# OATML-Markslab/ProteinGym

Measured on AMD Instinct MI355X. Metric: mutants scored/sec (ESM-1v 650M masked-marginal), higher is better.
Workload: dtype f16x3 (fp32 operands split into 2 fp16 planes, 3 fp16 MFMAs per product, fp32 accumulate)

## Files before the change

### proteingym_amd/csrc/api_ops.hip

```cpp
#include "model.h"

static inline float rebuild_split(unsigned short h, unsigned short l) {
    _Float16 a, b;
    memcpy(&a, &h, 2); memcpy(&b, &l, 2);
    return (float)a + (float)b * (1.0f / kLoScale);
}

extern "C" {

int pgmi_op_layernorm(int device, const float* x, const float* w, const float* b, int rows, int D, float eps, float* y) {
    if (!x || !w || !b || !y || rows <= 0 || D <= 0 || D % 4) { set_error("bad argument"); return PGMI_EINVAL; }
    if (pgmi_device_count() <= 0) { set_error("no HIP device visible"); return PGMI_ENODEV; }
    PGMI_HIP(hipSetDevice(device));
    std::vector<void*> pool;
    float *dx, *dw, *db, *dy;
    int rc = 0;
    if ((rc = dev_upload(pool, &dx, x, (size_t)rows * D)) || (rc = dev_upload(pool, &dw, w, (size_t)D)) ||
        (rc = dev_upload(pool, &db, b, (size_t)D)) || (rc = dev_alloc(pool, &dy, (size_t)rows * D))) {
        for (void* p : pool) hipFree(p);
        return rc;
    }
    launch_layernorm(dx, dw, db, rows, D, eps, dy, nullptr);
    hipError_t e = hipMemcpy(y, dy, (size_t)rows * D * 4, hipMemcpyDeviceToHost);
    for (void* p : pool) hipFree(p);
// ... 84 lines not shown
    if (er != hipSuccess) { set_error("moe op failed: %s", hipGetErrorString(er)); return PGMI_EHIP; }
    return PGMI_OK;
}

static GemmLaunch op_gemm(const unsigned short* a16, const W16& w16, const float* bias, int M, int N, int K, int variant) {
    GemmLaunch g;
    g.A = a16; g.W = w16.p; g.out_scale = w16.out_scale;
    g.bias = bias;
    g.M = M; g.N = N; g.K = K;
    g.variant = variant;
    return g;
}

int pgmi_op_gemm(int device, int precision, const float* A, const float* W, const float* bias, const float* residual,
                 int M, int N, int K, int epilogue, float* C) {
    if (!A || !W || !C || M <= 0 || N <= 0 || K <= 0) { set_error("bad argument"); return PGMI_EINVAL; }
    if (precision != PGMI_PREC_FP32 && precision != PGMI_PREC_F16X3 && precision != PGMI_PREC_BF16) { set_error("unknown precision %d", precision); return PGMI_EINVAL; }
    if (pgmi_device_count() <= 0) { set_error("no HIP device visible"); return PGMI_ENODEV; }
    PGMI_HIP(hipSetDevice(device));
    gemm_options_from_env();
    std::vector<void*> pool;
    float *dA, *dW = nullptr, *dB = nullptr, *dR = nullptr, *dC;
    int rc = 0;
    if ((rc = dev_upload(pool, &dA, A, (size_t)M * K)) ||
        (precision == PGMI_PREC_FP32 && (rc = dev_upload(pool, &dW, W, (size_t)N * K))) ||
        (bias && (rc = dev_upload(pool, &dB, bias, (size_t)N))) ||
        (residual && (rc = dev_upload(pool, &dR, residual, (size_t)M * N))) ||
        (rc = dev_alloc(pool, &dC, (size_t)M * N))) {
        for (void* p : pool) hipFree(p);
        return rc;
    }
    const int epi = epilogue & 255;
    const bool split_planes = (epilogue & 256) != 0;
    if (epi == EPI_SWIGLU && (!split_planes || precision != PGMI_PREC_F16X3 || (N % 64))) {
        for (void* p : pool) hipFree(p);
        set_error("SwiGLU GEMM op: precision f16x3 with the split-plane output (epilogue 4 + 256), N %% 64 == 0");
        return PGMI_EINVAL;
    }
    if (epi == EPI_RELU && precision != PGMI_PREC_F16X3) {
        for (void* p : pool) hipFree(p);
        set_error("ReLU GEMM op: precision f16x3 only");
        return PGMI_EINVAL;
    }
    if (split_planes && (precision == PGMI_PREC_FP32 || residual || (N % (precision == PGMI_PREC_F16X3 ? 32 : 4)))) {
        for (void* p : pool) hipFree(p);
        set_error("16-bit-plane GEMM op: f16x3 (N %% 32 == 0) or bf16 (N %% 4 == 0), no residual");
        return PGMI_EINVAL;
    }
    if (precision == PGMI_PREC_FP32) {
        rc = launch_gemm_f32(dA, dW, dB, dR, dC, M, N, K, epi, nullptr);
    } else {
        const bool bf = precision == PGMI_PREC_BF16;
        const int planes = bf ? 1 : 2;
        W16 w16;
        unsigned short* a16 = nullptr;
        rc = make_w16(pool, W, (size_t)N * K, (size_t)K, precision, nullptr, &w16);
        if (!rc) rc = dev_alloc(pool, &a16, (size_t)M * K * planes);
        if (!rc) {
            launch_split16(dA, (int64_t)M * K, 1.0f, bf ? 1 : 2, K, a16, nullptr);
            GemmLaunch g = op_gemm(a16, w16, dB, M, N, K, env_int("PGMI_GEMM_VARIANT", 0));
            g.epilogue = epi; g.bf = bf;
            if (split_planes) {
                unsigned short* c16 = nullptr;
                const int No = epi == EPI_SWIGLU ? N / 2 : N;
                rc = dev_alloc(pool, &c16, (size_t)M * N * 2);
                g.out16 = c16;
                if (!rc) rc = launch_gemm16(g);
                if (!rc) {
                    std::vector<unsigned short> h((size_t)M * N * 2);
                    hipError_t e2 = hipMemcpy(h.data(), c16, h.size() * 2, hipMemcpyDeviceToHost);
                    if (e2 != hipSuccess) { set_error("gemm op failed: %s", hipGetErrorString(e2)); rc = PGMI_EHIP; }
                    for (size_t m = 0; m < (size_t)M && !rc && bf; ++m)
                        for (int n = 0; n < N; ++n) {
                            const unsigned int u = (unsigned int)h[m * N + n] << 16;
                            memcpy(&C[m * N + n], &u, 4);
                        }
                    for (size_t m = 0; m < (size_t)M && !rc && !bf; ++m)
                        for (int n = 0; n < No; ++n) {
                            const size_t o = ki_off(m, n, No);
                            C[m * No + n] = rebuild_split(h[o], h[o + 32]);
                        }
                }
                for (void* p : pool) hipFree(p);
                return rc;
            }
            g.residual = dR; g.out32 = dC;
            rc = launch_gemm16(g);
        }
    }
    hipError_t e = hipMemcpy(C, dC, (size_t)M * N * 4, hipMemcpyDeviceToHost);
    for (void* p : pool) hipFree(p);
    if (rc) return rc;
    if (e != hipSuccess) { set_error("gemm op failed: %s", hipGetErrorString(e)); return PGMI_EHIP; }
    return PGMI_OK;
}

int pgmi_bench_gemm_ab(int device, int precision, int M, int N, int K, int epilogue, int split_out, const int* variants,
                       int n_variants, int rounds, int iters, double* ms_out) {
    if (M <= 0 || N <= 0 || K <= 0 || iters <= 0 || rounds <= 0 || n_variants <= 0 || !variants || !ms_out) { set_error("bad argument"); return PGMI_EINVAL; }
    if (pgmi_device_count() <= 0) { set_error("no HIP device visible"); return PGMI_ENODEV; }
    PGMI_HIP(hipSetDevice(device));
    gemm_options_from_env();
    std::vector<void*> pool;
    auto cleanup = [&]() { for (void* p : pool) hipFree(p); };
    std::vector<float> hA((size_t)M * K), hW((size_t)N * K), hb(N);
    unsigned int st = 12345u;
    auto rnd = [&]() { st = st * 1664525u + 1013904223u; return ((st >> 8) * (1.0f / 8388608.0f)) - 1.0f; };
    for (auto& v : hA) v = rnd();
    for (auto& v : hW) v = rnd() * 0.03f;
    for (auto& v : hb) v = rnd();
    float *dA, *dW = nullptr, *dB, *dC = nullptr;
    unsigned short *a16 = nullptr, *c16 = nullptr;
    int rc = 0;
    if ((rc = dev_upload(pool, &dA, hA.data(), hA.size())) || (rc = dev_upload(pool, &dB, hb.data(), hb.size()))) { cleanup(); return rc; }
    hipEvent_t e0, e1;
    PGMI_HIP(hipEventCreate(&e0));
// ... 674 lines not shown
```

### proteingym_amd/csrc/gemm16x_kernel.h

```cpp
#pragma once
#include <type_traits>

#include "common.h"

namespace pgmi {

typedef _Float16 h8 __attribute__((ext_vector_type(8)));
typedef _Float16 h4 __attribute__((ext_vector_type(4)));
typedef __bf16 b8 __attribute__((ext_vector_type(8)));
typedef unsigned int u32x4 __attribute__((ext_vector_type(4)));
typedef unsigned int u32x2 __attribute__((ext_vector_type(2)));

__device__ __forceinline__ f32x4 gelu_erf16(f32x4 x) {
    auto all = [](float v) { return f32x4{v, v, v, v}; };
    const f32x4 b = __builtin_elementwise_max(-__builtin_elementwise_abs(x), all(-6.0f));
    f32x4 q = __builtin_elementwise_fma(x, all(0.0f), all(3.309269596e-05f));
    q = __builtin_elementwise_fma(q, b, all(7.692188374e-04f));
    q = __builtin_elementwise_fma(q, b, all(8.080714382e-03f));
    q = __builtin_elementwise_fma(q, b, all(5.341210216e-02f));
    q = __builtin_elementwise_fma(q, b, all(-4.587709904e-01f));
    q = __builtin_elementwise_fma(q, b, all(1.151201725e+00f));
    q = __builtin_elementwise_fma(q, b, all(-9.999930859e-01f));
    const f32x4 e = {__builtin_amdgcn_exp2f(q[0]), __builtin_amdgcn_exp2f(q[1]), __builtin_amdgcn_exp2f(q[2]), __builtin_amdgcn_exp2f(q[3])};
    return __builtin_elementwise_fma(b, e, __builtin_elementwise_max(x, all(0.0f)));
// ... 128 lines not shown
            const int nwg = all_half ? n_items : tp.n_main, xcd = item & 7, q = nwg >> 3, r8 = nwg & 7;
            wgid = (xcd < r8 ? xcd * (q + 1) : r8 * (q + 1) + (xcd - r8) * q) + (item >> 3);
        } else {
            wgid = tp.n_main + ((item - tp.n_main) >> 1);
        }
        batch = 0;
        if (xm.tiles_per_batch) {
            batch = wgid / xm.tiles_per_batch;
            wgid -= batch * xm.tiles_per_batch;
            const int bi = batch % xm.batch_inner, bo = batch / xm.batch_inner;
            a_base = __builtin_amdgcn_readfirstlane((unsigned int)bi * xm.a_b0 + (unsigned int)bo * xm.a_b1);
            w_base = __builtin_amdgcn_readfirstlane((unsigned int)bi * xm.w_b0 + (unsigned int)bo * xm.w_b1);
            batch = __builtin_amdgcn_readfirstlane(batch);
        }
        int tm, tn;
        x_tile_coords(wgid, tp.tiles_m, tp.tiles_n, tm, tn, tp.group_m);
        half_item = all_half || (tp.half && item >= tp.n_main);
        a_ld = half_item ? LD / 2 : LD;
        m0 = __builtin_amdgcn_readfirstlane(all_half ? tm * (XBM / 2) : tm * XBM + (half_item ? ((item - tp.n_main) & 1) * (XBM / 2) : 0));
        n0 = __builtin_amdgcn_readfirstlane(tn * XBN);
#pragma unroll
        for (int i = 0; i < LD; ++i) {
            a_off[i] = (unsigned int)min(m0 + row_lo + 64 * i, M - 1) * a_row_bytes + (unsigned int)csrc * 16u;
            w_off[i] = (unsigned int)min(n0 + row_lo + 64 * i, N - 1) * w_row_bytes + (unsigned int)csrc * 16u;
        }
    };
    auto issue_tile = [&](int kt, int buf) {
        u32x4* base = lds + buf * X_STAGE + wave * 64;
        const int run = kt >> xm.k_run_log2, in_run = kt - (run << xm.k_run_log2);
        const int ka = (int)(a_base + (xm.a_run_bytes ? (unsigned int)run * xm.a_run_bytes + (unsigned int)in_run * 128u : (unsigned int)kt * 128u));
        const int kw = (int)(w_base + (xm.w_run_bytes ? (unsigned int)run * xm.w_run_bytes + (unsigned int)in_run * 128u : (unsigned int)kt * 128u));
#pragma unroll
        for (int i = 0; i < LD; ++i)
            if (i < a_ld)
                __builtin_amdgcn_raw_ptr_buffer_load_lds(rsA, (__attribute__((address_space(3))) void*)(base + XNT * i), 16, (int)a_off[i], ka, 0, 0);
#pragma unroll
        for (int i = 0; i < LD; ++i)
            __builtin_amdgcn_raw_ptr_buffer_load_lds(rsW, (__attribute__((address_space(3))) void*)(base + X_OP_CH + XNT * i), 16, (int)w_off[i], kw, 0, 0);
    };
    auto phase = [&]() {
        __builtin_amdgcn_sched_barrier(0);
        __builtin_amdgcn_s_waitcnt(0xC07F);
        __builtin_amdgcn_s_barrier();
        __builtin_amdgcn_sched_barrier(0);
    };
    auto phase_vm = [&]() {
        __builtin_amdgcn_sched_barrier(0);
        __builtin_amdgcn_s_waitcnt(0x0070);
        __builtin_amdgcn_s_barrier();
        __builtin_amdgcn_sched_barrier(0);
    };

    f32x4 acc[TN][TMX];
    u32x4 af[2][TMX / 2], wf[2][TN], whs[TN];
    const int fsw = (r >> 1) & 7;
    auto read_frags = [&](auto tmc, auto hc, const u32x4* Ab, const u32x4* Wb) {
        constexpr int TM = decltype(tmc)::value, TH = TM / 2, H = decltype(hc)::value;
// ... 38 lines not shown
#pragma unroll
        for (int j = 0; j < TN; ++j)
#pragma unroll
            for (int i = 0; i < TH; ++i) acc[j][H * TH + i] = mfma16x16<false>(whs[j], af[1][i], acc[j][H * TH + i]);
#pragma unroll
        for (int j = 0; j < TN; ++j)
#pragma unroll
            for (int i = 0; i < TH; ++i) acc[j][H * TH + i] = mfma16x16<false>(wf[0][j], af[0][i], acc[j][H * TH + i]);
        if constexpr (H == 0) {
#pragma unroll
            for (int k = 0; k < 4 * TN; ++k) {
                __builtin_amdgcn_sched_group_barrier(0x008, 1, 0);
                __builtin_amdgcn_sched_group_barrier(0x002, 1, 0);
            }
            __builtin_amdgcn_sched_group_barrier(0x008, 3 * TN * TH - 4 * TN, 0);
        }
    };
    using H0 = std::integral_constant<int, 0>;
    using H1 = std::integral_constant<int, 1>;

    int item = blockIdx.x;
    if (item >= n_items) return;
    decode(item);
    issue_tile(0, 0);
    auto run_item = [&](auto tmc) -> bool {
        constexpr int TM = decltype(tmc)::value;
        phase_vm();
#pragma unroll
        for (int j = 0; j < TN; ++j)
#pragma unroll
            for (int i = 0; i < TM; ++i)
#pragma unroll
                for (int v = 0; v < 4; ++v) acc[j][i][v] = 0.0f;
        int cur = 0;
        if (late) phase();
        for (int kt = 0; kt < nk; ++kt) {
            const u32x4* Ab = lds + cur * X_STAGE;
            const u32x4* Wb = Ab + X_OP_CH;
            __builtin_amdgcn_s_setprio(0);
            if (kt + 1 < nk) issue_tile(kt + 1, cur ^ 1);
            read_frags(tmc, H0{}, Ab, Wb);
            phase();
            __builtin_amdgcn_s_setprio(1);
            mfmas(tmc, H0{});
            phase();
            __builtin_amdgcn_s_setprio(0);
            read_frags(tmc, H1{}, Ab, Wb);
            if (late) phase_vm(); else phase();
            __builtin_amdgcn_s_setprio(1);
            mfmas(tmc, H1{});
            if (!late) phase_vm(); else phase();
            cur ^= 1;
        }
        __builtin_amdgcn_s_setprio(0);
        if (!late) phase();

        const int em0 = m0, en0 = n0, eb = batch;
        item += gridDim.x;
        const bool more = item < n_items;
        if (more) {
            decode(item);
            issue_tile(0, 0);
        }

        if constexpr (OUT == 2) {
            const int Dm = N / 3;
            const int nb = en0 + wn * 64;
            if (nb < N) {
            const int which = nb / Dm, hcol = nb - which * Dm, hh = hcol >> 6;
            constexpr int SPQ = 144;
            unsigned char* patch_q = patches + wave * (2 * 32 * SPQ);
            const bool staged_q = which < 2;
            f32x4 bq0[2], bq1[2];
#pragma unroll
            for (int g = 0; g < 2; ++g) {
                bq0[g] = *reinterpret_cast<const f32x4*>(bias + nb + 16 * g + 4 * kq);
                bq1[g] = *reinterpret_cast<const f32x4*>(bias + nb + 32 + 16 * g + 4 * kq);
            }
#pragma unroll
            for (int g = 0; g < 2; ++g) asm volatile("" :: "v"(bq0[g]), "v"(bq1[g]));
#pragma unroll
            for (int ib = 0; ib < TM / 2; ++ib) {
#pragma unroll
            for (int s = 0; s < 2; ++s) {
                const int i = 2 * ib + s, prow = 16 * s + r;
                const int m = em0 + (wm * TM + i) * 16 + r;
                const bool row_ok = m < M;
                if (!row_ok) continue;
                const int bb = m / qo.T, t = m - bb * qo.T;
                f32x4 rc[2], rs[2];
                if (which < 2 && qo.rotary) {
                    const int tr = (min(t, qo.T - 1) * qo.rot_halves + (hh % qo.rot_halves)) * 64;
#pragma unroll
                    for (int g = 0; g < 2; ++g) {
                        rc[g] = *reinterpret_cast<const f32x4*>(qo.cos_t + tr + 16 * g + 4 * kq);
                        rs[g] = *reinterpret_cast<const f32x4*>(qo.sin_t + tr + 16 * g + 4 * kq);
                    }
                }
#pragma unroll
                for (int g = 0; g < 2; ++g) {
                    const int d0 = 16 * g + 4 * kq;
// ... 47 lines not shown
                            c1p[0] = __builtin_bit_cast(unsigned short, a1);
                            c1p[qo.vt_plane] = __builtin_bit_cast(unsigned short, l1);
                        }
                    }
                }
            }
                if (staged_q) {
                    __builtin_amdgcn_wave_barrier();
                    const int m_base = em0 + (wm * TM + 2 * ib) * 16;
#pragma unroll
                    for (int k = 0; k < 4; ++k) {
                        const int q = lane + 64 * k, row = q >> 3, cc = q & 7;
                        const u32x4 vh = *reinterpret_cast<const u32x4*>(patch_q + row * SPQ + cc * 16);
                        const u32x4 vl = *reinterpret_cast<const u32x4*>(patch_q + (32 + row) * SPQ + cc * 16);
                        if (m_base + row < M) {
                            unsigned short* dst = Ch + (size_t)(m_base + row) * (2 * Dm) + (size_t)which * Dm + hcol + cc * 8;
                            *reinterpret_cast<u32x4*>(dst) = vh;
                            *reinterpret_cast<u32x4*>(dst + c_plane) = vl;
                        }
                    }
                    __builtin_amdgcn_wave_barrier();
                }
            }
            }
        } else if constexpr (OUT == 0) {
            unsigned char* patch = patches + wave * (32 * 128);
            const int cc = lane & 7, rq = lane >> 3;
            const unsigned int kOob = 0x80000000u;
            const unsigned int ldc = xm.ldc ? (unsigned int)xm.ldc : (unsigned int)N;
            const long long cb = xm.tiles_per_batch ? (long long)(eb % xm.batch_inner) * xm.c_b0 + (long long)(eb / xm.batch_inner) * xm.c_b1 : 0;
            const __amdgpu_buffer_rsrc_t rsC = __builtin_amdgcn_make_buffer_rsrc(Cf + cb, 0, (int)((unsigned int)M * ldc * 4u), 0x00020000);
            const __amdgpu_buffer_rsrc_t rsR = __builtin_amdgcn_make_buffer_rsrc(const_cast<float*>(residual ? residual : Cf) + cb, 0, (int)((unsigned int)M * ldc * 4u), 0x00020000);
            constexpr int NB = TN / 2;
            unsigned int coff[NB];
            f32x4 bv[NB];
#pragma unroll
            for (int j = 0; j < NB; ++j) {
                const int n = en0 + wn * 64 + j * 32 + cc * 4;
                coff[j] = n < N ? (unsigned int)n * 4u : kOob;
                bv[j] = (bias && n < N) ? *reinterpret_cast<const f32x4*>(bias + n) : f32x4{0.f, 0.f, 0.f, 0.f};
            }
#pragma unroll
            for (int j = 0; j < NB; ++j) asm volatile("" :: "v"(bv[j]));
            auto c_off = [&](int m, int j) -> int {
                return (int)((m < M && coff[j] != kOob) ? (unsigned int)m * ldc * 4u + coff[j] : kOob);
            };
            u32x4 rv[2][NB][4];
            auto load_residual = [&](int i, u32x4 (&dst)[NB][4]) {
                const int m_base = em0 + (wm * TM + 2 * i) * 16;
#pragma unroll
                for (int j = 0; j < NB; ++j)
#pragma unroll
                    for (int k = 0; k < 4; ++k)
                        dst[j][k] = __builtin_bit_cast(u32x4, __builtin_amdgcn_raw_buffer_load_b128(rsR, c_off(m_base + rq + 8 * k, j), 0, 0));
            };
            if (residual) load_residual(0, rv[0]);
#pragma unroll
            for (int i = 0; i < TM / 2; ++i) {
                const int m_base = em0 + (wm * TM + 2 * i) * 16;
                if (residual && i + 1 < TM / 2) load_residual(i + 1, rv[(i + 1) & 1]);
#pragma unroll
                for (int j = 0; j < NB; ++j) {
#pragma unroll
                    for (int s = 0; s < 2; ++s)
#pragma unroll
                        for (int u = 0; u < 2; ++u) {
                            const int prow = 16 * s + r;
                            *reinterpret_cast<f32x4*>(patch + prow * 128 + (((4 * u + kq) ^ (prow & 7)) << 4)) = acc[2 * j + u][2 * i + s];
                        }
                    __builtin_amdgcn_wave_barrier();
#pragma unroll
                    for (int k = 0; k < 4; ++k) {
                        const int row = rq + 8 * k;
                        const f32x4 a = *reinterpret_cast<const f32x4*>(patch + row * 128 + ((cc ^ (row & 7)) << 4));
                        f32x4 val;
#pragma unroll
                        for (int e = 0; e < 4; ++e) val[e] = fmaf(a[e], out_scale, bv[j][e]);
                        if (EPI == EPI_GELU) val = gelu_erf16(val);
                        if (EPI == EPI_GELU_TANH) val = gelu_tanh16(val);
                        if (EPI == EPI_SQRELU)
#pragma unroll
                        for (int e = 0; e < 4; ++e) { const float t = fmaxf(val[e], 0.0f); val[e] = t * t; }
                        if (EPI == EPI_RELU)
#pragma unroll
                        for (int e = 0; e < 4; ++e) val[e] = fmaxf(val[e], 0.0f);
                        if (residual) {
                            const f32x4 rr = __builtin_bit_cast(f32x4, rv[i & 1][j][k]);
#pragma unroll
                            for (int e = 0; e < 4; ++e) val[e] = rr[e] + val[e];
                        }
                        __builtin_amdgcn_raw_buffer_store_b128(__builtin_bit_cast(u32x4, val), rsC, c_off(m_base + row, j), 0, 0);
                    }
                    __builtin_amdgcn_wave_barrier();
                }
            }
        } else {
            if constexpr (BF) {
                constexpr int SPB = 144;
                const bool staged = (N % 8 == 0) && (en0 + (wn + 1) * 64 <= N);
                unsigned char* patch = patches + wave * (32 * SPB);
                f32x4 bvs[TN];
#pragma unroll
                for (int j = 0; j < TN; ++j) {
                    const int n = en0 + wn * 64 + 16 * j + 4 * kq;
                    bvs[j] = (bias && n < N) ? *reinterpret_cast<const f32x4*>(bias + n) : f32x4{0.f, 0.f, 0.f, 0.f};
                }
#pragma unroll
                for (int j = 0; j < TN; ++j) asm volatile("" :: "v"(bvs[j]));
#pragma unroll
                for (int ib = 0; ib < TM / 2; ++ib) {
#pragma unroll
                    for (int s = 0; s < 2; ++s) {
                    const int i = 2 * ib + s, prow = 16 * s + r;
                    const int m = em0 + (wm * TM + i) * 16 + r;
                    if (m >= M) continue;
#pragma unroll
                    for (int j = 0; j < TN; ++j) {
                            const int n = en0 + wn * 64 + 16 * j + 4 * kq;
                            if (n >= N) continue;
                            const f32x4 bv = bvs[j];
                            f32x4 val;
#pragma unroll
                            for (int e = 0; e < 4; ++e) val[e] = fmaf(acc[j][i][e], out_scale, bv[e]);
                            if (EPI == EPI_GELU) val = gelu_erf16(val);
                            if (EPI == EPI_GELU_TANH) val = gelu_tanh16(val);
                            if (EPI == EPI_SQRELU)
#pragma unroll
                            for (int e = 0; e < 4; ++e) { const float t = fmaxf(val[e], 0.0f); val[e] = t * t; }
                            if (EPI == EPI_RELU)
// ... 7 lines not shown
                        }
                    }
                    if (staged) {
                        __builtin_amdgcn_wave_barrier();
                        const int m_base = em0 + (wm * TM + 2 * ib) * 16;
                        const size_t ncol0 = (size_t)en0 + (size_t)wn * 64;
#pragma unroll
                        for (int k = 0; k < 4; ++k) {
                            const int q = lane + 64 * k, row = q >> 3, cc = q & 7;
                            const u32x4 v = *reinterpret_cast<const u32x4*>(patch + row * SPB + cc * 16);
                            if (m_base + row < M) *reinterpret_cast<u32x4*>(Ch + (size_t)(m_base + row) * (size_t)N + ncol0 + cc * 8) = v;
                        }
                        __builtin_amdgcn_wave_barrier();
                    }
                }
            } else if constexpr (EPI == EPI_SWIGLU) {
            constexpr int SPS = 144;
            const int Nh = N >> 1, nw = en0 + wn * 64;
            if (nw < N) {
            unsigned char* patch = patches + wave * (32 * SPS);
            f32x4 bvs[TN];
#pragma unroll
            for (int j = 0; j < TN; ++j)
                bvs[j] = bias ? *reinterpret_cast<const f32x4*>(bias + nw + 16 * j + 4 * kq) : f32x4{0.f, 0.f, 0.f, 0.f};
#pragma unroll
            for (int j = 0; j < TN; ++j) asm volatile("" :: "v"(bvs[j]));
#pragma unroll
            for (int ib = 0; ib < TM / 2; ++ib) {
#pragma unroll
                for (int s = 0; s < 2; ++s) {
                    const int i = 2 * ib + s, prow = 16 * s + r;
                    if (em0 + (wm * TM + i) * 16 + r >= M) continue;
#pragma unroll
                    for (int j = 0; j < 2; ++j) {
                        f32x4 g, u;
#pragma unroll
                        for (int e = 0; e < 4; ++e) {
                            g[e] = fmaf(acc[j][i][e], out_scale, bvs[j][e]);
                            u[e] = fmaf(acc[j + 2][i][e], out_scale, bvs[j + 2][e]);
                        }
                        const f32x4 val = silu16(g) * u;
                        h4 hi, lo;
#pragma unroll
                        for (int e = 0; e < 4; ++e) {
                            _Float16 a, b;
                            split_act(val[e], a, b);
                            hi[e] = a;
                            lo[e] = b;
                        }
                        unsigned char* cell = patch + prow * SPS + (16 * j + 4 * kq) * 2;
                        lds_put(cell, hi);
                        lds_put(cell + 64, lo);
                    }
                }
                __builtin_amdgcn_wave_barrier();
                const int m_base = em0 + (wm * TM + 2 * ib) * 16;
#pragma unroll
                for (int k = 0; k < 4; ++k) {
                    const int q = lane + 64 * k, row = q >> 3, cc = q & 7;
                    const u32x4 v = *reinterpret_cast<const u32x4*>(patch + row * SPS + cc * 16);
                    if (m_base + row < M) *reinterpret_cast<u32x4*>(Ch + (size_t)(m_base + row) * (2 * (size_t)Nh) + (size_t)nw + cc * 8) = v;
                }
                __builtin_amdgcn_wave_barrier();
            }
            }
            } else {
            constexpr int SP = 272;
            const bool staged = (N % 8 == 0) && (en0 + (wn + 1) * 64 <= N);
            unsigned char* patch = patches + wave * (32 * SP);
            f32x4 bvs[TN];
#pragma unroll
            for (int j = 0; j < TN; ++j) {
                const int n = en0 + wn * 64 + 16 * j + 4 * kq;
                bvs[j] = (bias && n < N) ? *reinterpret_cast<const f32x4*>(bias + n) : f32x4{0.f, 0.f, 0.f, 0.f};
            }
#pragma unroll
            for (int j = 0; j < TN; ++j) asm volatile("" :: "v"(bvs[j]));
#pragma unroll
            for (int ib = 0; ib < TM / 2; ++ib) {
#pragma unroll
                for (int s = 0; s < 2; ++s) {
                const int i = 2 * ib + s, prow = 16 * s + r;
                const int m = em0 + (wm * TM + i) * 16 + r;
                if (m >= M) continue;
#pragma unroll
                for (int j = 0; j < TN; ++j) {
                    {
                        const int c = 16 * j + 4 * kq;
                        const int n = en0 + wn * 64 + c;
                        if (n >= N) continue;
                        const f32x4 bv = bvs[j];
                        f32x4 val;
#pragma unroll
                        for (int e = 0; e < 4; ++e) val[e] = fmaf(acc[j][i][e], out_scale, bv[e]);
                        if (EPI == EPI_GELU) val = gelu_erf16(val);
                        if (EPI == EPI_GELU_TANH) val = gelu_tanh16(val);
                        if (EPI == EPI_SQRELU)
#pragma unroll
                        for (int e = 0; e < 4; ++e) { const float t = fmaxf(val[e], 0.0f); val[e] = t * t; }
                        if (EPI == EPI_RELU)
#pragma unroll
                        for (int e = 0; e < 4; ++e) val[e] = fmaxf(val[e], 0.0f);
                        {
                            h4 hi, lo;
#pragma unroll
                            for (int e = 0; e < 4; ++e) {
                                _Float16 a, b;
                                split_act(val[e], a, b);
                                hi[e] = a;
                                lo[e] = b;
                            }
                            if (staged) {
                                unsigned char* cell = patch + prow * SP + (c >> 5) * 128 + (c & 31) * 2;
                                lds_put(cell, hi);
                                lds_put(cell + 64, lo);
                            } else {
                                unsigned short* dst = Ch + ki_off((size_t)m, n, N);
                                *reinterpret_cast<h4*>(dst) = hi;
                                *reinterpret_cast<h4*>(dst + 32) = lo;
                            }
                        }
                    }
                }
                }
                if (staged) {
                    __builtin_amdgcn_wave_barrier();
                    const int m_base = em0 + (wm * TM + 2 * ib) * 16;
                    const size_t ncol0 = (size_t)en0 + (size_t)wn * 64;
#pragma unroll
                    for (int k = 0; k < 8; ++k) {
                        const int q = lane + 64 * k;
                        const int row = q >> 4, cc = q & 15;
                        const u32x4 v = *reinterpret_cast<const u32x4*>(patch + row * SP + cc * 16);
                        if (m_base + row < M) {
                            if (xm.o_ld)
                                *reinterpret_cast<u32x4*>(Ch + ((size_t)(m_base + row) + (ncol0 >> 6) * (size_t)xm.o_rows_per_n64) * (2 * (size_t)xm.o_ld) +
                                                          (size_t)eb * (size_t)xm.o_col_per_batch * 2 + cc * 8) = v;
                            else
                                *reinterpret_cast<u32x4*>(Ch + (size_t)(m_base + row) * (2 * (size_t)N) + ncol0 * 2 + cc * 8) = v;
                        }
                    }
                    __builtin_amdgcn_wave_barrier();
                }
            }
            }
        }
        return more;
    };
    using Full = std::integral_constant<int, TMX>;
    using Half = std::integral_constant<int, TMX / 2>;
    while (true) {
        bool more;
        if constexpr (OUT != 2) more = half_item ? run_item(Half{}) : run_item(Full{});
        else more = run_item(Full{});
        if (!more) break;
    }
}

}
```

### proteingym_amd/csrc/gemm_f16.hip

```cpp
#include <stdlib.h>
#include <string.h>
#include <algorithm>
#include <mutex>

#include "common.h"
#include "gemm16x_kernel.h"

namespace pgmi {

constexpr int kMaxDevices = 64;
static int g_num_cus[kMaxDevices];
static std::mutex g_xdev_mu;

static int x_num_cus() {
    int dev = 0;
    if (hipGetDevice(&dev) != hipSuccess || dev < 0 || dev >= kMaxDevices) dev = 0;
    std::lock_guard<std::mutex> lk(g_xdev_mu);
    int& n = g_num_cus[dev];
    if (!n) {
        hipDeviceProp_t prop;
        if (hipGetDeviceProperties(&prop, dev) == hipSuccess) n = prop.multiProcessorCount;
        if (n <= 0) n = 256;
        n -= n % 8;
        if (n <= 0) n = 8;
// ... 42 lines not shown
    inst<EPI_GELU, X_OUT_F32, false, true>(),      inst<EPI_GELU, X_OUT_16, false, true>(),
    inst<EPI_SQRELU, X_OUT_F32, false, true>(),    inst<EPI_SQRELU, X_OUT_16, false, true>(),
    inst<EPI_GELU_TANH, X_OUT_F32, false, true>(), inst<EPI_GELU_TANH, X_OUT_16, false, true>(),
    inst<EPI_NONE, X_OUT_F32, true>(),             inst<EPI_NONE, X_OUT_16, true>(),
};

static int launch_x(const GemmLaunch& g, int out, bool xm, size_t c_plane, int G, int n_items, const TilePlan& tp, const QkvOut& qo,
                    const XMap& xmap) {
    const GemmInst* k = nullptr;
    for (const GemmInst& i : kGemmInst)
        if (i.epi == g.epilogue && i.out == out && i.xm == xm && i.bf == g.bf) { k = &i; break; }
    if (!k) {
        set_error("gemm16: no kernel for epilogue %d, output kind %d, xmap %d, bf16 %d", g.epilogue, out, (int)xm, (int)g.bf);
        return PGMI_EINVAL;
    }
    hipError_t e = hipFuncSetAttribute(reinterpret_cast<const void*>(k->fn), hipFuncAttributeMaxDynamicSharedMemorySize, (int)X_LDS_BYTES);
    if (e != hipSuccess) { set_error("hipFuncSetAttribute: %s", hipGetErrorString(e)); return PGMI_EHIP; }
    hipLaunchKernelGGL(k->fn, dim3(std::min(G, n_items)), dim3(XNT), X_LDS_BYTES, g.stream, g.A, g.W, g.bias, g.residual, g.out32, g.out16,
                       c_plane, g.M, g.N, g.K, g.out_scale, tp, qo, xmap);
    PGMI_HIP(hipGetLastError());
    return PGMI_OK;
}

static int launch_gemm16x_one(const GemmLaunch& g, int group_m) {
    const int M = g.M, N = g.N, K = g.K;
    const bool qkv = g.qkv.vt16 != nullptr;
    const unsigned long long eb = g.bf ? 2ull : 4ull;
    TilePlan tp{};
    tp.group_m = group_m > 0 ? group_m : ((N + XBN - 1) / XBN >= kWideTilesN ? kGroupMWide : kGroupM);
    tp.tiles_m = (M + XBM - 1) / XBM;
    tp.tiles_n = (N + XBN - 1) / XBN;
    const int T = tp.tiles_m * tp.tiles_n, G = x_num_cus();
    tp.n_main = T;
    if ((unsigned long long)std::max(M, N) * (unsigned long long)K * eb >= (1ull << 32) ||
        (g.out32 && (unsigned long long)M * (unsigned long long)N * 4ull >= (1ull << 31))) {
        set_error("gemm16x: operand of %d x %d split elements (or %d x %d outputs) exceeds the 32-bit offset range", std::max(M, N), K, M, N);
        return PGMI_EINVAL;
    }
    const int rem = T % G;
    if (g_opt.half_tail && !qkv && rem > 0 && 2 * rem <= G) {
        tp.n_main = T - rem; tp.half = 1; tp.n_tail = 2 * rem;
    }
    QkvOut qo{};
    if (qkv) qo = QkvOut{g.qkv.vt16, g.qkv.vt_plane, g.qkv.cos_t, g.qkv.sin_t, g.qkv.T, g.qkv.H, (g.qkv.T + 31) / 32 * 32, g.qkv.rotary, g.qkv.rot_halves};
    return launch_x(g, qkv ? X_OUT_QKV : g.out16 ? X_OUT_16 : X_OUT_F32, false, qkv ? g.qkv.qk_plane : 0, G, tp.n_main + tp.n_tail, tp, qo, XMap{});
}

int launch_gemm16_ex(const unsigned short* A, const unsigned short* W, float* Cf, unsigned short* Ch, int M, int N, int K,
                     float out_scale, XMap xm, int nbatch, hipStream_t s) {
    if (M <= 0 || N <= 0 || K <= 0 || (K % 64) != 0 || (N % 4) != 0 || (!Cf && !Ch) || (Cf && Ch) || nbatch < 1 ||
        (Ch && (N % 64) != 0) || (xm.a_run_bytes && (K / 32) % (1 << xm.k_run_log2) != 0)) {
        set_error("gemm16_ex: unsupported shape/args M=%d N=%d K=%d batches=%d", M, N, K, nbatch);
        return PGMI_EINVAL;
    }
    TilePlan tp{};
    tp.group_m = kGroupM;
    const int rows_last = M % XBM;
    const bool all_half = rows_last > 0 && rows_last <= XBM / 2;
// ... 3 lines not shown
    xm.tiles_per_batch = per;
    if (xm.batch_inner < 1) xm.batch_inner = 1;
    if (all_half) { tp.half = 2; tp.n_main = 0; tp.n_tail = T; } else { tp.n_main = T; }
    GemmLaunch g;
    g.A = A; g.W = W; g.out_scale = out_scale;
    g.out32 = Cf; g.out16 = Ch;
    g.M = M; g.N = N; g.K = K;
    g.stream = s;
    return launch_x(g, Ch ? X_OUT_16 : X_OUT_F32, true, 0, G, T, tp, QkvOut{}, xm);
}

static int launch_gemm16x(const GemmLaunch& g) {
    const int M = g.M, N = g.N, K = g.K, group_m = gemm_group_m(g.variant);
    const bool qkv = g.qkv.vt16 != nullptr;
    const unsigned long long lim = (1ull << 32) - 1;
    const unsigned long long eb = g.bf ? 2ull : 4ull;
    if ((unsigned long long)N * (unsigned long long)K * eb > lim) {
        set_error("gemm16x: weight of %d x %d split elements exceeds the 32-bit offset range", N, K);
        return PGMI_EINVAL;
    }
    const long long test_rows = g_opt.max_rows;
    long long max_rows = (long long)(lim / ((unsigned long long)K * eb));
    if (g.out32) max_rows = std::min(max_rows, (long long)(((1ull << 31) - 1) / ((unsigned long long)N * 4ull)));
    if (test_rows > 0) max_rows = std::min(max_rows, test_rows);
    if (M <= max_rows) return launch_gemm16x_one(g, group_m);
    long long per = qkv ? (max_rows / g.qkv.T) * g.qkv.T : (max_rows / XBM) * XBM;
    if (per <= 0) per = qkv ? 0 : max_rows;
    if (per <= 0) { set_error("gemm16x: one sequence of %d tokens x K = %d exceeds the 32-bit offset range", g.qkv.T, K); return PGMI_EINVAL; }
    const size_t n_out16 = qkv ? (size_t)(2 * (N / 3)) : (size_t)(g.bf ? 1 : 2) * (g.epilogue == EPI_SWIGLU ? (size_t)N / 2 : (size_t)N);
    for (long long m0 = 0; m0 < M; m0 += per) {
        GemmLaunch c = g;
        c.M = (int)std::min<long long>(per, M - m0);
        c.A = g.A + (size_t)m0 * (size_t)K * (g.bf ? 1 : 2);
        if (g.residual) c.residual = g.residual + (size_t)m0 * N;
        if (g.out32) c.out32 = g.out32 + (size_t)m0 * N;
        if (g.out16) c.out16 = g.out16 + (size_t)m0 * n_out16;
        if (qkv) c.qkv.vt16 = g.qkv.vt16 + (size_t)(m0 / g.qkv.T) * (size_t)g.qkv.H * kHeadDim * (size_t)((g.qkv.T + 31) / 32 * 32);
        const int rc = launch_gemm16x_one(c, group_m);
        if (rc) return rc;
    }
    return PGMI_OK;
}

int launch_gemm16(const GemmLaunch& g) {
    const int M = g.M, N = g.N, K = g.K;
    const int k_step = g.bf ? 64 : 32;
    if (g.qkv.vt16) {
        const int D = N / 3, T = g.qkv.T;
        if (M <= 0 || K <= 0 || D <= 0 || N != 3 * D || (K % k_step) || (D % 64) || T <= 0 || M % T || g.qkv.rot_halves < 1 || !g.out16 || g.out32 ||
            g.residual || g.epilogue != EPI_NONE) {
            set_error("gemm16_qkv: unsupported shape M=%d D=%d K=%d T=%d", M, D, K, T);
            return PGMI_EINVAL;
// ... 45 lines not shown
```

Before: 18410.

## Prefetch next tile during GEMM epilogue and use buffer stores for split output

In the persistent f16x3 GEMM kernel, the first K-tile loads of the next work item are now issued inside each epilogue, right after the bias loads, so the global-to-LDS fetch overlaps the output writes. To allow this without branches, out-of-range A rows and idle blocks get sentinel offsets, and bias is read through a buffer resource that returns zeros out of range. The staged split-plane epilogue now writes with bounds-checked buffer stores, adding a 32-bit offset limit to the host-side row chunking. The residual path is specialised at compile time, and guard-band checks in the test op look for writes past row M.

```diff
diff --git a/proteingym_amd/csrc/api_ops.hip b/proteingym_amd/csrc/api_ops.hip
--- a/proteingym_amd/csrc/api_ops.hip
+++ b/proteingym_amd/csrc/api_ops.hip
@@ -130,14 +130,23 @@
     std::vector<void*> pool;
     float *dA, *dW = nullptr, *dB = nullptr, *dR = nullptr, *dC;
     int rc = 0;
+    constexpr size_t kGuardRows = 256;
+    auto guard_fill = [&](void* band, size_t bytes) { return hipMemset(band, 0xff, bytes) == hipSuccess; };
+    auto guard_intact = [&](const void* band, size_t bytes) {
+        std::vector<unsigned char> h(bytes);
+        if (hipMemcpy(h.data(), band, bytes, hipMemcpyDeviceToHost) != hipSuccess) return false;
+        for (unsigned char b : h) if (b != 0xff) return false;
+        return true;
+    };
     if ((rc = dev_upload(pool, &dA, A, (size_t)M * K)) ||
         (precision == PGMI_PREC_FP32 && (rc = dev_upload(pool, &dW, W, (size_t)N * K))) ||
         (bias && (rc = dev_upload(pool, &dB, bias, (size_t)N))) ||
         (residual && (rc = dev_upload(pool, &dR, residual, (size_t)M * N))) ||
-        (rc = dev_alloc(pool, &dC, (size_t)M * N))) {
+        (rc = dev_alloc(pool, &dC, ((size_t)M + kGuardRows) * N))) {
         for (void* p : pool) hipFree(p);
         return rc;
     }
+    if (!guard_fill(dC + (size_t)M * N, kGuardRows * N * 4)) { for (void* p : pool) hipFree(p); set_error("gemm op: hipMemset failed"); return PGMI_EHIP; }
     const int epi = epilogue & 255;
     const bool split_planes = (epilogue & 256) != 0;
     if (epi == EPI_SWIGLU && (!split_planes || precision != PGMI_PREC_F16X3 || (N % 64))) {
@@ -171,9 +180,11 @@
             if (split_planes) {
                 unsigned short* c16 = nullptr;
                 const int No = epi == EPI_SWIGLU ? N / 2 : N;
-                rc = dev_alloc(pool, &c16, (size_t)M * N * 2);
+                rc = dev_alloc(pool, &c16, ((size_t)M + kGuardRows) * N * 2);
                 g.out16 = c16;
+                if (!rc && !guard_fill(c16 + (size_t)M * N * 2, kGuardRows * N * 4)) { set_error("gemm op: hipMemset failed"); rc = PGMI_EHIP; }
                 if (!rc) rc = launch_gemm16(g);
+                if (!rc && !guard_intact(c16 + (size_t)M * N * 2, kGuardRows * N * 4)) { set_error("gemm op: the kernel wrote past row M of its 16-bit output"); rc = PGMI_EHIP; }
                 if (!rc) {
                     std::vector<unsigned short> h((size_t)M * N * 2);
                     hipError_t e2 = hipMemcpy(h.data(), c16, h.size() * 2, hipMemcpyDeviceToHost);
@@ -197,9 +208,11 @@
         }
     }
     hipError_t e = hipMemcpy(C, dC, (size_t)M * N * 4, hipMemcpyDeviceToHost);
+    const bool intact = rc || e != hipSuccess || guard_intact(dC + (size_t)M * N, kGuardRows * N * 4);
     for (void* p : pool) hipFree(p);
     if (rc) return rc;
     if (e != hipSuccess) { set_error("gemm op failed: %s", hipGetErrorString(e)); return PGMI_EHIP; }
+    if (!intact) { set_error("gemm op: the kernel wrote past row M of its fp32 output"); return PGMI_EHIP; }
     return PGMI_OK;
 }
 
diff --git a/proteingym_amd/csrc/gemm16x_kernel.h b/proteingym_amd/csrc/gemm16x_kernel.h
--- a/proteingym_amd/csrc/gemm16x_kernel.h
+++ b/proteingym_amd/csrc/gemm16x_kernel.h
@@ -174,17 +174,18 @@
 #pragma unroll
         for (int i = 0; i < LD; ++i) {
             a_off[i] = (unsigned int)min(m0 + row_lo + 64 * i, M - 1) * a_row_bytes + (unsigned int)csrc * 16u;
+            if (i >= a_ld) a_off[i] = 0xfffffff0u;
             w_off[i] = (unsigned int)min(n0 + row_lo + 64 * i, N - 1) * w_row_bytes + (unsigned int)csrc * 16u;
         }
     };
-    auto issue_tile = [&](int kt, int buf) {
+    auto issue_tile = [&](int kt, int buf, auto all) {
         u32x4* base = lds + buf * X_STAGE + wave * 64;
         const int run = kt >> xm.k_run_log2, in_run = kt - (run << xm.k_run_log2);
         const int ka = (int)(a_base + (xm.a_run_bytes ? (unsigned int)run * xm.a_run_bytes + (unsigned int)in_run * 128u : (unsigned int)kt * 128u));
         const int kw = (int)(w_base + (xm.w_run_bytes ? (unsigned int)run * xm.w_run_bytes + (unsigned int)in_run * 128u : (unsigned int)kt * 128u));
 #pragma unroll
         for (int i = 0; i < LD; ++i)
-            if (i < a_ld)
+            if (decltype(all)::value || i < a_ld)
                 __builtin_amdgcn_raw_ptr_buffer_load_lds(rsA, (__attribute__((address_space(3))) void*)(base + XNT * i), 16, (int)a_off[i], ka, 0, 0);
 #pragma unroll
         for (int i = 0; i < LD; ++i)
@@ -269,7 +270,7 @@
     int item = blockIdx.x;
     if (item >= n_items) return;
     decode(item);
-    issue_tile(0, 0);
+    issue_tile(0, 0, std::false_type{});
     auto run_item = [&](auto tmc) -> bool {
         constexpr int TM = decltype(tmc)::value;
         phase_vm();
@@ -285,7 +286,7 @@
             const u32x4* Ab = lds + cur * X_STAGE;
             const u32x4* Wb = Ab + X_OP_CH;
             __builtin_amdgcn_s_setprio(0);
-            if (kt + 1 < nk) issue_tile(kt + 1, cur ^ 1);
+            if (kt + 1 < nk) issue_tile(kt + 1, cur ^ 1, std::false_type{});
             read_frags(tmc, H0{}, Ab, Wb);
             phase();
             __builtin_amdgcn_s_setprio(1);
@@ -305,10 +306,21 @@
         const int em0 = m0, en0 = n0, eb = batch;
         item += gridDim.x;
         const bool more = item < n_items;
-        if (more) {
-            decode(item);
-            issue_tile(0, 0);
-        }
+        const __amdgpu_buffer_rsrc_t rsB = __builtin_amdgcn_make_buffer_rsrc(const_cast<float*>(bias), 0, bias ? N * 4 : 0, 0x00020000);
+        auto load_bias = [&](int n) -> f32x4 {
+            return __builtin_bit_cast(f32x4, __builtin_amdgcn_raw_buffer_load_b128(rsB, n * 4, 0, 0));
+        };
+        auto next_item = [&]() {
+            __builtin_amdgcn_sched_barrier(0);
+            if (more) decode(item);
+#pragma unroll
+            for (int i = 0; i < LD; ++i) {
+                if (!more) a_off[i] = w_off[i] = 0xfffffff0u;
+                asm volatile("" : "+v"(a_off[i]), "+v"(w_off[i]));
+            }
+            issue_tile(0, 0, std::true_type{});
+            __builtin_amdgcn_sched_barrier(0);
+        };
 
         if constexpr (OUT == 2) {
             const int Dm = N / 3;
@@ -321,9 +333,10 @@
             f32x4 bq0[2], bq1[2];
 #pragma unroll
             for (int g = 0; g < 2; ++g) {
-                bq0[g] = *reinterpret_cast<const f32x4*>(bias + nb + 16 * g + 4 * kq);
-                bq1[g] = *reinterpret_cast<const f32x4*>(bias + nb + 32 + 16 * g + 4 * kq);
-            }
+                bq0[g] = load_bias(nb + 16 * g + 4 * kq);
+                bq1[g] = load_bias(nb + 32 + 16 * g + 4 * kq);
+            }
+            next_item();
 #pragma unroll
             for (int g = 0; g < 2; ++g) asm volatile("" :: "v"(bq0[g]), "v"(bq1[g]));
 #pragma unroll
@@ -417,10 +430,14 @@
                     __builtin_amdgcn_wave_barrier();
                 }
             }
+            } else {
+                next_item();
             }
         } else if constexpr (OUT == 0) {
             unsigned char* patch = patches + wave * (32 * 128);
-            const int cc = lane & 7, rq = lane >> 3;
+            int le = lane;
+            asm volatile("" : "+v"(le));
+            const int cc = le & 7, rq = le >> 3, er = le & 15, ekq = le >> 4;
             const unsigned int kOob = 0x80000000u;
             const unsigned int ldc = xm.ldc ? (unsigned int)xm.ldc : (unsigned int)N;
             const long long cb = xm.tiles_per_batch ? (long long)(eb % xm.batch_inner) * xm.c_b0 + (long long)(eb / xm.batch_inner) * xm.c_b1 : 0;
@@ -433,62 +450,67 @@
             for (int j = 0; j < NB; ++j) {
                 const int n = en0 + wn * 64 + j * 32 + cc * 4;
                 coff[j] = n < N ? (unsigned int)n * 4u : kOob;
-                bv[j] = (bias && n < N) ? *reinterpret_cast<const f32x4*>(bias + n) : f32x4{0.f, 0.f, 0.f, 0.f};
-            }
-#pragma unroll
-            for (int j = 0; j < NB; ++j) asm volatile("" :: "v"(bv[j]));
+                bv[j] = load_bias(n);
+            }
             auto c_off = [&](int m, int j) -> int {
-                return (int)((m < M && coff[j] != kOob) ? (unsigned int)m * ldc * 4u + coff[j] : kOob);
+                return (int)(m < M ? (unsigned int)m * ldc * 4u + coff[j] : kOob);
             };
-            u32x4 rv[2][NB][4];
-            auto load_residual = [&](int i, u32x4 (&dst)[NB][4]) {
-                const int m_base = em0 + (wm * TM + 2 * i) * 16;
-#pragma unroll
-                for (int j = 0; j < NB; ++j)
-#pragma unroll
-                    for (int k = 0; k < 4; ++k)
-                        dst[j][k] = __builtin_bit_cast(u32x4, __builtin_amdgcn_raw_buffer_load_b128(rsR, c_off(m_base + rq + 8 * k, j), 0, 0));
+            auto blocks = [&](auto has_res) {
+                constexpr bool RES = decltype(has_res)::value;
+                u32x4 rv[2][NB][4];
+                auto load_residual = [&](int i, u32x4 (&dst)[NB][4]) {
+                    const int m_base = em0 + (wm * TM + 2 * i) * 16;
+#pragma unroll
+                    for (int j = 0; j < NB; ++j)
+#pragma unroll
+                        for (int k = 0; k < 4; ++k)
+                            dst[j][k] = __builtin_bit_cast(u32x4, __builtin_amdgcn_raw_buffer_load_b128(rsR, c_off(m_base + rq + 8 * k, j), 0, 0));
+                };
+                if constexpr (RES) load_residual(0, rv[0]);
+                next_item();
+#pragma unroll
+                for (int j = 0; j < NB; ++j) asm volatile("" :: "v"(bv[j]));
+#pragma unroll
+                for (int i = 0; i < TM / 2; ++i) {
+                    const int m_base = em0 + (wm * TM + 2 * i) * 16;
+#pragma unroll
+                    for (int j = 0; j < NB; ++j) {
+                        if constexpr (RES) if (j == (EPI == EPI_NONE ? 0 : 1) && i + 1 < TM / 2) load_residual(i + 1, rv[(i + 1) & 1]);
+#pragma unroll
+                        for (int s = 0; s < 2; ++s)
+#pragma unroll
+                            for (int u = 0; u < 2; ++u) {
+                                const int prow = 16 * s + er;
+                                *reinterpret_cast<f32x4*>(patch + prow * 128 + (((4 * u + ekq) ^ (prow & 7)) << 4)) = acc[2 * j + u][2 * i + s];
+                            }
+                        __builtin_amdgcn_wave_barrier();
+#pragma unroll
+                        for (int k = 0; k < 4; ++k) {
+                            const int row = rq + 8 * k;
+                            const f32x4 a = *reinterpret_cast<const f32x4*>(patch + row * 128 + ((cc ^ (row & 7)) << 4));
+                            f32x4 val;
+#pragma unroll
+                            for (int e = 0; e < 4; ++e) val[e] = fmaf(a[e], out_scale, bv[j][e]);
+                            if (EPI == EPI_GELU) val = gelu_erf16(val);
+                            if (EPI == EPI_GELU_TANH) val = gelu_tanh16(val);
+                            if (EPI == EPI_SQRELU)
+#pragma unroll
+                            for (int e = 0; e < 4; ++e) { const float t = fmaxf(val[e], 0.0f); val[e] = t * t; }
+                            if (EPI == EPI_RELU)
+#pragma unroll
+                            for (int e = 0; e < 4; ++e) val[e] = fmaxf(val[e], 0.0f);
+                            if constexpr (RES) {
+                                const f32x4 rr = __builtin_bit_cast(f32x4, rv[i & 1][j][k]);
+#pragma unroll
+                                for (int e = 0; e < 4; ++e) val[e] = rr[e] + val[e];
+                            }
+                            __builtin_amdgcn_raw_buffer_store_b128(__builtin_bit_cast(u32x4, val), rsC, c_off(m_base + row, j), 0, 0);
+                        }
+                        __builtin_amdgcn_wave_barrier();
+                    }
+                }
             };
-            if (residual) load_residual(0, rv[0]);
-#pragma unroll
-            for (int i = 0; i < TM / 2; ++i) {
-                const int m_base = em0 + (wm * TM + 2 * i) * 16;
-                if (residual && i + 1 < TM / 2) load_residual(i + 1, rv[(i + 1) & 1]);
-#pragma unroll
-                for (int j = 0; j < NB; ++j) {
-#pragma unroll
-                    for (int s = 0; s < 2; ++s)
-#pragma unroll
-                        for (int u = 0; u < 2; ++u) {
-                            const int prow = 16 * s + r;
-                            *reinterpret_cast<f32x4*>(patch + prow * 128 + (((4 * u + kq) ^ (prow & 7)) << 4)) = acc[2 * j + u][2 * i + s];
-                        }
-                    __builtin_amdgcn_wave_barrier();
-#pragma unroll
-                    for (int k = 0; k < 4; ++k) {
-                        const int row = rq + 8 * k;
-                        const f32x4 a = *reinterpret_cast<const f32x4*>(patch + row * 128 + ((cc ^ (row & 7)) << 4));
-                        f32x4 val;
-#pragma unroll
-                        for (int e = 0; e < 4; ++e) val[e] = fmaf(a[e], out_scale, bv[j][e]);
-                        if (EPI == EPI_GELU) val = gelu_erf16(val);
-                        if (EPI == EPI_GELU_TANH) val = gelu_tanh16(val);
-                        if (EPI == EPI_SQRELU)
-#pragma unroll
-                        for (int e = 0; e < 4; ++e) { const float t = fmaxf(val[e], 0.0f); val[e] = t * t; }
-                        if (EPI == EPI_RELU)
-#pragma unroll
-                        for (int e = 0; e < 4; ++e) val[e] = fmaxf(val[e], 0.0f);
-                        if (residual) {
-                            const f32x4 rr = __builtin_bit_cast(f32x4, rv[i & 1][j][k]);
-#pragma unroll
-                            for (int e = 0; e < 4; ++e) val[e] = rr[e] + val[e];
-                        }
-                        __builtin_amdgcn_raw_buffer_store_b128(__builtin_bit_cast(u32x4, val), rsC, c_off(m_base + row, j), 0, 0);
-                    }
-                    __builtin_amdgcn_wave_barrier();
-                }
-            }
+            if (residual) blocks(std::true_type{}); else blocks(std::false_type{});
         } else {
             if constexpr (BF) {
                 constexpr int SPB = 144;
@@ -498,8 +520,9 @@
 #pragma unroll
                 for (int j = 0; j < TN; ++j) {
                     const int n = en0 + wn * 64 + 16 * j + 4 * kq;
-                    bvs[j] = (bias && n < N) ? *reinterpret_cast<const f32x4*>(bias + n) : f32x4{0.f, 0.f, 0.f, 0.f};
-                }
+                    bvs[j] = load_bias(n);
+                }
+                next_item();
 #pragma unroll
                 for (int j = 0; j < TN; ++j) asm volatile("" :: "v"(bvs[j]));
 #pragma unroll
@@ -553,7 +576,8 @@
             f32x4 bvs[TN];
 #pragma unroll
             for (int j = 0; j < TN; ++j)
-                bvs[j] = bias ? *reinterpret_cast<const f32x4*>(bias + nw + 16 * j + 4 * kq) : f32x4{0.f, 0.f, 0.f, 0.f};
+                bvs[j] = load_bias(nw + 16 * j + 4 * kq);
+            next_item();
 #pragma unroll
             for (int j = 0; j < TN; ++j) asm volatile("" :: "v"(bvs[j]));
 #pragma unroll
@@ -594,6 +618,8 @@
                 }
                 __builtin_amdgcn_wave_barrier();
             }
+            } else {
+                next_item();
             }
             } else {
             constexpr int SP = 272;
@@ -603,10 +629,65 @@
 #pragma unroll
             for (int j = 0; j < TN; ++j) {
                 const int n = en0 + wn * 64 + 16 * j + 4 * kq;
-                bvs[j] = (bias && n < N) ? *reinterpret_cast<const f32x4*>(bias + n) : f32x4{0.f, 0.f, 0.f, 0.f};
-            }
+                bvs[j] = load_bias(n);
+            }
+            next_item();
 #pragma unroll
             for (int j = 0; j < TN; ++j) asm volatile("" :: "v"(bvs[j]));
+            auto group = [&](int i, int j, h4& hi, h4& lo) {
+                f32x4 val;
+#pragma unroll
+                for (int e = 0; e < 4; ++e) val[e] = fmaf(acc[j][i][e], out_scale, bvs[j][e]);
+                if (EPI == EPI_GELU) val = gelu_erf16(val);
+                if (EPI == EPI_GELU_TANH) val = gelu_tanh16(val);
+                if (EPI == EPI_SQRELU)
+#pragma unroll
+                for (int e = 0; e < 4; ++e) { const float t = fmaxf(val[e], 0.0f); val[e] = t * t; }
+                if (EPI == EPI_RELU)
+#pragma unroll
+                for (int e = 0; e < 4; ++e) val[e] = fmaxf(val[e], 0.0f);
+#pragma unroll
+                for (int e = 0; e < 4; ++e) {
+                    _Float16 a, b;
+                    split_act(val[e], a, b);
+                    hi[e] = a;
+                    lo[e] = b;
+                }
+            };
+            if (!XM && staged) {
+                const __amdgpu_buffer_rsrc_t rsH = __builtin_amdgcn_make_buffer_rsrc(Ch, 0, (int)((unsigned int)M * (unsigned int)N * 4u), 0x00020000);
+                const unsigned int kOob = 0x80000000u, row_bytes = (unsigned int)N * 4u;
+                int le = lane;
+                asm volatile("" : "+v"(le));
+                const int er = le & 15, ekq = le >> 4;
+                const unsigned int col_b = (unsigned int)(en0 + wn * 64) * 4u + (unsigned int)er * 16u;
+#pragma unroll
+                for (int ib = 0; ib < TM / 2; ++ib) {
+#pragma unroll
+                    for (int s = 0; s < 2; ++s)
+#pragma unroll
+                        for (int j = 0; j < TN; ++j) {
+                            const int c = 16 * j + 4 * ekq;
+                            h4 hi, lo;
+                            group(2 * ib + s, j, hi, lo);
+                            unsigned char* cell = patch + (16 * s + er) * SP + (c >> 5) * 128 + (c & 31) * 2;
+                            lds_put(cell, hi);
+                            lds_put(cell + 64, lo);
+                        }
+                    __builtin_amdgcn_wave_barrier();
+                    const int m_base = em0 + (wm * TM + 2 * ib) * 16;
+                    u32x4 v[8];
+#pragma unroll
+                    for (int k = 0; k < 8; ++k) v[k] = *reinterpret_cast<const u32x4*>(patch + (ekq + 4 * k) * SP + er * 16);
+#pragma unroll
+                    for (int k = 0; k < 8; ++k) {
+                        const int m = m_base + ekq + 4 * k;
+                        __builtin_amdgcn_raw_buffer_store_b128(v[k], rsH, (int)(m < M ? (unsigned int)m * row_bytes + col_b : kOob), 0, 0);
+                    }
+                    __builtin_amdgcn_wave_barrier();
+                }
+            } else {
+            const bool st = XM && staged;
 #pragma unroll
             for (int ib = 0; ib < TM / 2; ++ib) {
 #pragma unroll
@@ -616,45 +697,23 @@
                 if (m >= M) continue;
 #pragma unroll
                 for (int j = 0; j < TN; ++j) {
-                    {
-                        const int c = 16 * j + 4 * kq;
-                        const int n = en0 + wn * 64 + c;
-                        if (n >= N) continue;
-                        const f32x4 bv = bvs[j];
-                        f32x4 val;
-#pragma unroll
-                        for (int e = 0; e < 4; ++e) val[e] = fmaf(acc[j][i][e], out_scale, bv[e]);
-                        if (EPI == EPI_GELU) val = gelu_erf16(val);
-                        if (EPI == EPI_GELU_TANH) val = gelu_tanh16(val);
-                        if (EPI == EPI_SQRELU)
-#pragma unroll
-                        for (int e = 0; e < 4; ++e) { const float t = fmaxf(val[e], 0.0f); val[e] = t * t; }
-                        if (EPI == EPI_RELU)
-#pragma unroll
-                        for (int e = 0; e < 4; ++e) val[e] = fmaxf(val[e], 0.0f);
-                        {
-                            h4 hi, lo;
-#pragma unroll
-                            for (int e = 0; e < 4; ++e) {
-                                _Float16 a, b;
-                                split_act(val[e], a, b);
-                                hi[e] = a;
-                                lo[e] = b;
-                            }
-                            if (staged) {
-                                unsigned char* cell = patch + prow * SP + (c >> 5) * 128 + (c & 31) * 2;
-                                lds_put(cell, hi);
-                                lds_put(cell + 64, lo);
-                            } else {
-                                unsigned short* dst = Ch + ki_off((size_t)m, n, N);
-                                *reinterpret_cast<h4*>(dst) = hi;
-                                *reinterpret_cast<h4*>(dst + 32) = lo;
-                            }
-                        }
-                    }
-                }
-                }
-                if (staged) {
+                    const int c = 16 * j + 4 * kq;
+                    const int n = en0 + wn * 64 + c;
+                    if (n >= N) continue;
+                    h4 hi, lo;
+                    group(i, j, hi, lo);
+                    if (st) {
+                        unsigned char* cell = patch + prow * SP + (c >> 5) * 128 + (c & 31) * 2;
+                        lds_put(cell, hi);
+                        lds_put(cell + 64, lo);
+                    } else {
+                        unsigned short* dst = Ch + ki_off((size_t)m, n, N);
+                        *reinterpret_cast<h4*>(dst) = hi;
+                        *reinterpret_cast<h4*>(dst + 32) = lo;
+                    }
+                }
+                }
+                if (st) {
                     __builtin_amdgcn_wave_barrier();
                     const int m_base = em0 + (wm * TM + 2 * ib) * 16;
                     const size_t ncol0 = (size_t)en0 + (size_t)wn * 64;
@@ -673,6 +732,7 @@
                     }
                     __builtin_amdgcn_wave_barrier();
                 }
+            }
             }
             }
         }
diff --git a/proteingym_amd/csrc/gemm_f16.hip b/proteingym_amd/csrc/gemm_f16.hip
--- a/proteingym_amd/csrc/gemm_f16.hip
+++ b/proteingym_amd/csrc/gemm_f16.hip
@@ -88,6 +88,12 @@
     return PGMI_OK;
 }
 
+static size_t out16_row_halfs(const GemmLaunch& g) {
+    if (g.qkv.vt16) return (size_t)(2 * (g.N / 3));
+    return (size_t)(g.bf ? 1 : 2) * (g.epilogue == EPI_SWIGLU ? (size_t)g.N / 2 : (size_t)g.N);
+}
+static bool out16_buffer_stores(const GemmLaunch& g) { return g.out16 && !g.qkv.vt16 && !g.bf && g.epilogue != EPI_SWIGLU; }
+
 static int launch_gemm16x_one(const GemmLaunch& g, int group_m) {
     const int M = g.M, N = g.N, K = g.K;
     const bool qkv = g.qkv.vt16 != nullptr;
@@ -99,7 +105,8 @@
     const int T = tp.tiles_m * tp.tiles_n, G = x_num_cus();
     tp.n_main = T;
     if ((unsigned long long)std::max(M, N) * (unsigned long long)K * eb >= (1ull << 32) ||
-        (g.out32 && (unsigned long long)M * (unsigned long long)N * 4ull >= (1ull << 31))) {
+        (g.out32 && (unsigned long long)M * (unsigned long long)N * 4ull >= (1ull << 31)) ||
+        (out16_buffer_stores(g) && (unsigned long long)M * (unsigned long long)out16_row_halfs(g) * 2ull >= (1ull << 31))) {
         set_error("gemm16x: operand of %d x %d split elements (or %d x %d outputs) exceeds the 32-bit offset range", std::max(M, N), K, M, N);
         return PGMI_EINVAL;
     }
@@ -149,12 +156,13 @@
     const long long test_rows = g_opt.max_rows;
     long long max_rows = (long long)(lim / ((unsigned long long)K * eb));
     if (g.out32) max_rows = std::min(max_rows, (long long)(((1ull << 31) - 1) / ((unsigned long long)N * 4ull)));
+    const size_t n_out16 = out16_row_halfs(g);
+    if (out16_buffer_stores(g)) max_rows = std::min(max_rows, (long long)(((1ull << 31) - 1) / ((unsigned long long)n_out16 * 2ull)));
     if (test_rows > 0) max_rows = std::min(max_rows, test_rows);
     if (M <= max_rows) return launch_gemm16x_one(g, group_m);
     long long per = qkv ? (max_rows / g.qkv.T) * g.qkv.T : (max_rows / XBM) * XBM;
     if (per <= 0) per = qkv ? 0 : max_rows;
     if (per <= 0) { set_error("gemm16x: one sequence of %d tokens x K = %d exceeds the 32-bit offset range", g.qkv.T, K); return PGMI_EINVAL; }
-    const size_t n_out16 = qkv ? (size_t)(2 * (N / 3)) : (size_t)(g.bf ? 1 : 2) * (g.epilogue == EPI_SWIGLU ? (size_t)N / 2 : (size_t)N);
     for (long long m0 = 0; m0 < M; m0 += per) {
         GemmLaunch c = g;
         c.M = (int)std::min<long long>(per, M - m0);
```

After: 18570 (median of 6 runs). Within noise of the previous version (+0.9%).
